# modassarrana89/authorino

Hardware: AMD Instinct MI355X
Metric: request×rule evals/sec (+ allow/deny decisions/sec, % HBM roofline) (higher is better)
Workload: dtype u8

## Files before the change

authorino_amd/csrc/ajx_api.cpp:

```cpp
#include <cstdio>
#include <cstring>
#include <memory>
#include <string>

#include "ajx_host.h"
#include "ajx_blob.h"
#include "ajx_kernels.h"

thread_local AjxLastError ajx_last_error;

struct EndEvent {
    hipEvent_t ev = nullptr;
    ~EndEvent() {
        if (ev) (void)hipEventDestroy(ev);
    }
};

struct Workspace {
    hipStream_t stream = nullptr;
    uint64_t id = 0;
    uint32_t refs = 0;
    bool retired = false;
    std::mutex mu;
    hipEvent_t ev0 = nullptr, ev1 = nullptr;
    std::shared_ptr<EndEvent> end;
    const uint8_t** d_sets = nullptr;
    ajx::DeviceBuf sets_dev;
    ajx::PinnedBuf sets_host;
    uint32_t sets_cap = 0;
    uint32_t sets_slot = 0;
    hipEvent_t sets_ev[2] = {nullptr, nullptr};
    bool sets_ev_rec[2] = {false, false};
    std::vector<const uint8_t*> last_sets;
    ajx::PtrTable progs;
    ajx::DeviceBuf slow;
    bool cnt_zero = false, exact_published = false;
    ajx::DeviceBuf rows;
    ajx::DeviceBuf perm;
    ajx::DeviceBuf tout;
    const authjx_ruleset* rows_rs = nullptr;
    uint32_t rows_n = 0, rows_stride = 0;
    const uint32_t* rows_perm = nullptr;
    bool rows_wave = false;
    bool ran = false;
};

namespace {
std::mutex g_reg_mu;
std::vector<std::pair<uint64_t, std::shared_ptr<EndEvent>>> g_reg;
uint64_t g_next_ws = 1;

Workspace* workspace_of(authjx_ctx* ctx, hipStream_t s) {
    for (Workspace* w : ctx->ws)
        if (w->stream == s) return w;
    Workspace* w = new Workspace();
    w->stream = s;
    w->end = std::make_shared<EndEvent>();
    if (hipEventCreate(&w->ev0) != hipSuccess || hipEventCreate(&w->end->ev) != hipSuccess) {
        if (w->ev0) (void)hipEventDestroy(w->ev0);
        delete w;
        return nullptr;
    }
    w->ev1 = w->end->ev;
    {
        std::lock_guard<std::mutex> lock(g_reg_mu);
        w->id = g_next_ws++;
        g_reg.push_back({w->id, w->end});
    }
    ctx->ws.push_back(w);
    return w;
}

void destroy_workspace(Workspace* w) {
    if (w->ran) (void)hipEventSynchronize(w->ev1);
    {
        std::lock_guard<std::mutex> lock(g_reg_mu);
        for (size_t i = 0; i < g_reg.size(); i++)
            if (g_reg[i].first == w->id) {
                g_reg.erase(g_reg.begin() + (long)i);
                break;
            }
    }
    for (int k = 0; k < 2; k++) {
        if (w->sets_ev[k]) (void)hipEventDestroy(w->sets_ev[k]);
        if (w->progs.ev[k]) (void)hipEventDestroy(w->progs.ev[k]);
    }
    if (w->ev0) (void)hipEventDestroy(w->ev0);
    delete w;
}

Workspace* ws_ref(Workspace* w) {
// ... 3 lines not shown
void ws_unref(authjx_ctx* ctx, Workspace* w) {
    bool dead;
    {
        std::lock_guard<std::mutex> g(ctx->mu);
        dead = --w->refs == 0 && w->retired;
    }
    if (dead) destroy_workspace(w);
}

int ensure_sets(Workspace* w, int device, const authjx_ruleset* const* sets, uint32_t n_sets,
                const uint8_t* const* d_pre = nullptr) {
    std::vector<const uint8_t*> ptrs(n_sets);
    for (uint32_t i = 0; i < n_sets; i++) {
        if (!sets[i] || sets[i]->device != device) return AUTHJX_EINVAL;
        ptrs[i] = sets[i]->d_blob.data();
    }
    if (d_pre) {
        w->d_sets = const_cast<const uint8_t**>(d_pre);
        w->last_sets.clear();
        return AUTHJX_OK;
    }
    if (ptrs == w->last_sets) return AUTHJX_OK;
    if (n_sets > w->sets_cap) {
        const uint32_t cap = n_sets < 64 ? 64 : n_sets;
        w->d_sets = nullptr;
        w->sets_cap = 0;
        w->sets_ev_rec[0] = w->sets_ev_rec[1] = false;
        HIP_OK(w->sets_dev.reserve(2 * cap * sizeof(uint8_t*), w->stream));
        HIP_OK(w->sets_host.reserve(2 * cap * sizeof(uint8_t*), w->stream));
        for (int k = 0; k < 2; k++)
            if (!w->sets_ev[k]) HIP_OK(hipEventCreateWithFlags(&w->sets_ev[k], hipEventDisableTiming));
        w->sets_cap = cap;
    }
    const uint32_t k = w->d_sets ? 1u - w->sets_slot : 0u;
    if (w->sets_ev_rec[k]) HIP_OK(hipEventSynchronize(w->sets_ev[k]));
    const uint8_t** h = w->sets_host.as<const uint8_t*>() + (size_t)k * w->sets_cap;
    const uint8_t** dv = w->sets_dev.as<const uint8_t*>() + (size_t)k * w->sets_cap;
    std::memcpy(h, ptrs.data(), n_sets * sizeof(uint8_t*));
    HIP_OK(hipMemcpyAsync(dv, h, n_sets * sizeof(uint8_t*), hipMemcpyHostToDevice, w->stream));
    w->sets_slot = k;
    w->d_sets = dv;
    w->last_sets = ptrs;
    return AUTHJX_OK;
}

int ensure_work(Workspace* w, uint32_t n, uint32_t row_stride) {
    const size_t slow_bytes = ((size_t)n + ajx::kStreamCounterWords) * sizeof(uint32_t);
    const size_t perm_bytes = ajx::PermBuf::words(n) * sizeof(uint32_t);
    const size_t rows_bytes = (size_t)((n + 63u) & ~63u) * row_stride * sizeof(uint64_t);
    if (slow_bytes <= w->slow.capacity() && perm_bytes <= w->perm.capacity() && rows_bytes <= w->rows.capacity())
        return AUTHJX_OK;
    w->rows_rs = nullptr;
    if (slow_bytes > w->slow.capacity()) w->cnt_zero = w->exact_published = false;
    HIP_OK(w->slow.reserve(slow_bytes, w->stream));
    HIP_OK(w->perm.reserve(perm_bytes, w->stream));
    HIP_OK(w->rows.reserve(rows_bytes, w->stream));
    return AUTHJX_OK;
}

struct WsLock {
    authjx_ctx* ctx;
    Workspace* w = nullptr;
    std::unique_lock<std::mutex> lock;
    WsLock(authjx_ctx* c, void* stream) : ctx(c) {
        {
            std::lock_guard<std::mutex> g(ctx->mu);
            w = ws_ref(workspace_of(ctx, stream ? (hipStream_t)stream : ctx->stream));
        }
        if (w) {
            lock = std::unique_lock<std::mutex>(w->mu);
            std::lock_guard<std::mutex> g(ctx->mu);
            if (!w->retired) ctx->last_ws = w;
        }
    }
    ~WsLock() {
        if (!w) return;
        lock.unlock();
        ws_unref(ctx, w);
    }
    WsLock(const WsLock&) = delete;
    WsLock& operator=(const WsLock&) = delete;
};

struct LastWs {
    authjx_ctx* ctx;
    Workspace* w = nullptr;
    int force_scan = 0;
    explicit LastWs(authjx_ctx* c) : ctx(c) {
        std::lock_guard<std::mutex> g(ctx->mu);
        w = ws_ref(ctx->last_ws);
        force_scan = ctx->force_scan;
    }
    ~LastWs() {
        if (w) ws_unref(ctx, w);
    }
    LastWs(const LastWs&) = delete;
    LastWs& operator=(const LastWs&) = delete;
};

int batch_done(Workspace* w, const authjx_ruleset* const* sets, uint32_t n_sets) {
    HIP_OK(hipEventRecord(w->ev1, w->stream));
    if (w->sets_ev[w->sets_slot]) {
        HIP_OK(hipEventRecord(w->sets_ev[w->sets_slot], w->stream));
        w->sets_ev_rec[w->sets_slot] = true;
    }
    w->ran = true;
    for (uint32_t i = 0; i < n_sets; i++) const_cast<authjx_ruleset*>(sets[i])->note_use(w->id);
    return AUTHJX_OK;
}
// ... 120 lines not shown
    ajx::PtrTable& t = w->progs;
    if (t.last.empty() || !std::equal(t.last.begin(), t.last.end(), ptrs, ptrs + n)) {
        if (n > t.cap) {
            const uint32_t cap = n < 64 ? 64 : n;
            t.cap = 0;
            t.last.clear();
            t.rec[0] = t.rec[1] = false;
            HIP_OK(t.dev.reserve(2 * (size_t)cap * sizeof(uint8_t*), w->stream));
            HIP_OK(t.host.reserve(2 * (size_t)cap * sizeof(uint8_t*), w->stream));
            for (int k = 0; k < 2; k++)
                if (!t.ev[k]) HIP_OK(hipEventCreateWithFlags(&t.ev[k], hipEventDisableTiming));
            t.cap = cap;
        }
        const uint32_t k = t.last.empty() ? 0u : 1u - t.slot;
        if (t.rec[k]) HIP_OK(hipEventSynchronize(t.ev[k]));
        const uint8_t** h = t.host.as<const uint8_t*>() + (size_t)k * t.cap;
        std::memcpy(h, ptrs, n * sizeof(uint8_t*));
        HIP_OK(hipMemcpyAsync(t.dev.as<const uint8_t*>() + (size_t)k * t.cap, h, n * sizeof(uint8_t*),
                              hipMemcpyHostToDevice, w->stream));
        t.slot = k;
        t.last.assign(ptrs, ptrs + n);
    }
    HIP_OK(launch(t.dev.as<const uint8_t*>() + (size_t)t.slot * t.cap, w->stream));
    HIP_OK(hipEventRecord(t.ev[t.slot], w->stream));
    t.rec[t.slot] = true;
    HIP_OK(hipEventRecord(w->ev1, w->stream));
    w->ran = true;
    return AUTHJX_OK;
}

int eval_device(authjx_ctx* ctx, const authjx_ruleset* const* sets, uint32_t n_sets, const uint32_t* d_set_of_req,
                const uint8_t* d_arena, const uint64_t* d_offs, const uint32_t* d_lens, uint32_t n,
                uint8_t* d_out_tristate, int32_t* d_out_err_idx, uint64_t* d_out_bitmap, uint32_t bitmap_stride_words,
                void* stream, const uint8_t* const* d_sets_pre) {
    if (!ctx || !sets || n_sets == 0 || (n && (!d_arena || !d_offs || !d_lens || !d_out_tristate)))
        return AUTHJX_EINVAL;
    if (n_sets > 1 && !d_set_of_req) return AUTHJX_EINVAL;
    if (n_sets == 1) d_set_of_req = nullptr;
    uint32_t need_words = 0;
    for (uint32_t i = 0; i < n_sets; i++) {
        if (!sets[i] || sets[i]->c.n_trees != sets[0]->c.n_trees) return AUTHJX_EINVAL;
        need_words = std::max(need_words, (sets[i]->c.n_patterns + 63) / 64);
    }
    if (d_out_bitmap && bitmap_stride_words < need_words) return AUTHJX_EINVAL;
    const ajx::PlanIn in = plan_in(ctx, sets, n_sets, n, d_out_bitmap != nullptr);
    const ajx::EvalPlan plan = ajx::plan_eval(in);
    WsLock wl(ctx, stream);
    Workspace* w = wl.w;
    if (!w) return AUTHJX_EDEVICE;
    hipStream_t s = w->stream;
    HIP_OK(hipSetDevice(ctx->device));
    int rc = ensure_sets(w, ctx->device, sets, n_sets, d_sets_pre);
    if (rc != AUTHJX_OK) return rc;
    if (plan.path != ajx::kPathExact && (rc = ensure_work(w, n, plan.rows_stride)) != AUTHJX_OK) return rc;
    HIP_OK(hipEventRecord(w->ev0, s));
    w->rows_rs = plan.keep_rows ? sets[0] : nullptr;
    w->rows_n = n;
    w->rows_stride = plan.rows_stride;
    w->rows_perm = nullptr;
    w->rows_wave = true;
    bool cnt_zero = w->cnt_zero;
    w->cnt_zero = w->exact_published = false;
    uint32_t* const slow = w->slow.as<uint32_t>();
    const ajx::Batch batch{w->d_sets, d_set_of_req, d_arena, d_offs, d_lens, n};
    const ajx::Results res{d_out_tristate, d_out_err_idx, d_out_bitmap, bitmap_stride_words};
    if (plan.path == ajx::kPathExact) {
        HIP_OK(ajx::launch_eval_scan(batch, res, plan.mods != 0, s));
    } else if (plan.path == ajx::kPathStream) {
        const ajx::Work work{w->rows.as<uint64_t>(), plan.rows_stride, slow, ajx::stream_slow_ids(slow)};
        HIP_OK(ajx::launch_eval_stream(batch, res, work, plan, in.max_blob, in.max_rec,
                                       ajx::PermBuf{w->perm.as<uint32_t>(), n}.stage_list(), &cnt_zero, s));
        w->cnt_zero = w->exact_published = cnt_zero;
    } else {
        const uint32_t* perm = nullptr;
        uint32_t* pos_of = nullptr;
        const ajx::PermBuf order{w->perm.as<uint32_t>(), n};
        if (plan.len_order) {
            if (plan.want_pos_of) {
                HIP_OK(w->tout.reserve(ajx::tout_bytes(n, plan.n_out, plan.tout_bm ? bitmap_stride_words : 0u), s));
                pos_of = order.pos_of();
            }
            HIP_OK(ajx::launch_len_order(d_lens, n, order.hist(), order.perm(), pos_of, s));
            perm = order.perm();
        }
        w->rows_perm = perm;
        const ajx::Work work{w->rows.as<uint64_t>(), plan.rows_stride, slow, slow + 1};
        HIP_OK(ajx::launch_eval_fast(batch, res, work, plan, perm, pos_of, pos_of ? w->tout.data() : nullptr, s));
    }
    return batch_done(w, sets, n_sets);
}

extern "C" {

#ifndef AJX_SRC_HASH
#define AJX_SRC_HASH "unknown"
#endif
const char* authjx_build_hash(void) { return AJX_SRC_HASH; }

int authjx_device_count(void) {
    int n = 0;
    if (hipGetDeviceCount(&n) != hipSuccess) return 0;
    return n;
}

int authjx_init(int device, authjx_ctx** out) {
    if (!out) return AUTHJX_EINVAL;
    *out = nullptr;
    int n = authjx_device_count();
    if (device < 0 || device >= n) return AUTHJX_EDEVICE;
    HIP_OK(hipSetDevice(device));
    authjx_ctx* c = new authjx_ctx();
    c->device = device;
    if (hipStreamCreateWithFlags(&c->stream, hipStreamNonBlocking) != hipSuccess) {
        delete c;
        return AUTHJX_EDEVICE;
    }
    *out = c;
    return AUTHJX_OK;
}

void authjx_shutdown(authjx_ctx* ctx) {
    if (!ctx) return;
    std::vector<authjx_batcher*> live;
    {
        std::lock_guard<std::mutex> g(ctx->mu);
        live = ctx->batchers;
    }
    for (authjx_batcher* b : live) authjx_batcher_destroy(b);
    (void)hipSetDevice(ctx->device);
    if (ctx->stream) (void)hipStreamSynchronize(ctx->stream);
    for (Workspace* w : ctx->ws) destroy_workspace(w);
    if (ctx->stream) (void)hipStreamDestroy(ctx->stream);
    delete ctx;
}

int authjx_release_stream(authjx_ctx* ctx, void* stream) {
    if (!ctx || !stream || (hipStream_t)stream == ctx->stream) return AUTHJX_EINVAL;
    (void)hipSetDevice(ctx->device);
    retire_stream(ctx, (hipStream_t)stream);
    return AUTHJX_OK;
}

// ... 37 lines not shown
}

uint32_t authjx_ruleset_patterns(const authjx_ruleset* rs) { return rs ? rs->c.n_patterns : 0; }
uint32_t authjx_ruleset_selectors(const authjx_ruleset* rs) { return rs ? rs->c.n_selectors : 0; }

size_t authjx_pattern_error(const authjx_ruleset* rs, uint32_t i, char* buf, size_t cap) {
    if (!rs || i >= rs->c.n_patterns) return 0;
    const std::string& e = rs->c.pattern_error[i];
    if (buf && cap) std::snprintf(buf, cap, "%s", e.c_str());
    return e.size();
}

int authjx_eval_batch_device(authjx_ctx* ctx, const authjx_ruleset* const* sets, uint32_t n_sets,
                             const uint32_t* d_set_of_req, const uint8_t* d_arena, const uint64_t* d_offs,
                             const uint32_t* d_lens, uint32_t n, uint8_t* d_out_tristate, int32_t* d_out_err_idx,
                             uint64_t* d_out_bitmap, uint32_t bitmap_stride_words, void* stream) {
    return eval_device(ctx, sets, n_sets, d_set_of_req, d_arena, d_offs, d_lens, n, d_out_tristate, d_out_err_idx,
                       d_out_bitmap, bitmap_stride_words, stream, nullptr);
}

static_assert(sizeof(authjx_value) == 12, "authjx_value is three u32 words on the device");

int authjx_select_batch_device(authjx_ctx* ctx, const authjx_ruleset* const* sets, uint32_t n_sets,
                               const uint32_t* d_set_of_req, const uint8_t* d_arena, const uint64_t* d_offs,
                               const uint32_t* d_lens, uint32_t n, authjx_value* d_out_values,
                               uint32_t values_stride, void* stream) {
    return authjx_select_text_batch_device(ctx, sets, n_sets, d_set_of_req, d_arena, d_offs, d_lens, n, d_out_values,
                                           values_stride, nullptr, 0, stream);
}

int authjx_select_text_batch_device(authjx_ctx* ctx, const authjx_ruleset* const* sets, uint32_t n_sets,
                                    const uint32_t* d_set_of_req, const uint8_t* d_arena, const uint64_t* d_offs,
                                    const uint32_t* d_lens, uint32_t n, authjx_value* d_out_values,
                                    uint32_t values_stride, uint8_t* d_out_text, uint32_t text_stride, void* stream) {
    if (!ctx || !sets || n_sets == 0 || (n && (!d_arena || !d_offs || !d_lens || !d_out_values)))
        return AUTHJX_EINVAL;
    if (d_out_text && text_stride == 0) return AUTHJX_EINVAL;
    if (n_sets > 1 && !d_set_of_req) return AUTHJX_EINVAL;
    if (n_sets == 1) d_set_of_req = nullptr;
    for (uint32_t i = 0; i < n_sets; i++)
        if (!sets[i] || sets[i]->c.n_patterns > values_stride) return AUTHJX_EINVAL;
    const ajx::PlanIn in = plan_in(ctx, sets, n_sets, n, false);
    const uint32_t row_stride = 1 + in.max_sel;
    WsLock wl(ctx, stream);
    Workspace* w = wl.w;
    if (!w) return AUTHJX_EDEVICE;
    hipStream_t s = w->stream;
    HIP_OK(hipSetDevice(ctx->device));
    int rc = ensure_sets(w, ctx->device, sets, n_sets);
    if (rc != AUTHJX_OK) return rc;
    const bool exact = in.force_scan != 0;
    w->rows_rs = nullptr;
    w->cnt_zero = w->exact_published = false;
    if (!exact && (rc = ensure_work(w, n, row_stride)) != AUTHJX_OK) return rc;
    const uint32_t* perm = nullptr;
    if (!exact && in.len_sort && n_sets == 1 && n >= 4096) {
        const ajx::PermBuf order{w->perm.as<uint32_t>(), n};
        HIP_OK(ajx::launch_len_order(d_lens, n, order.hist(), order.perm(), nullptr, s));
        perm = order.perm();
    }
    const uint32_t shared_bytes =
        (n_sets == 1 && sets[0]->blob_bytes <= ajx::kMaxSharedBlobBytes) ? sets[0]->blob_bytes : 0u;
    uint32_t* const slow = w->slow.as<uint32_t>();
    const ajx::Batch batch{w->d_sets, d_set_of_req, d_arena, d_offs, d_lens, n};
    const ajx::Values values{reinterpret_cast<uint32_t*>(d_out_values), values_stride, d_out_text, text_stride};
    const ajx::Work work{exact ? nullptr : w->rows.as<uint64_t>(), row_stride, slow, slow + 1};
    HIP_OK(ajx::launch_select(batch, shared_bytes, values, work, perm, s));
    return batch_done(w, sets, n_sets);
}

int authjx_select_from_eval_device(authjx_ctx* ctx, const authjx_ruleset* rs, uint32_t first_pattern,
                                   const uint8_t* d_arena, const uint64_t* d_offs, const uint32_t* d_lens,
                                   uint32_t n, authjx_value* d_out_values, uint32_t values_stride, void* stream) {
    if (!ctx || !rs || values_stride == 0 || (n && (!d_arena || !d_offs || !d_lens || !d_out_values)))
        return AUTHJX_EINVAL;
    if (first_pattern + values_stride > rs->c.n_patterns) return AUTHJX_EINVAL;
    WsLock wl(ctx, stream);
    Workspace* w = wl.w;
    if (!w) return AUTHJX_EDEVICE;
    if (w->rows_rs != rs || w->rows_n != n || !rows_hold_patterns(rs, first_pattern, values_stride))
        return AUTHJX_EINVAL;
    hipStream_t s = w->stream;
    HIP_OK(hipSetDevice(ctx->device));
    const authjx_ruleset* one[1] = {rs};
    int rc = ensure_sets(w, ctx->device, one, 1);
    if (rc != AUTHJX_OK) return rc;
    const ajx::Batch batch{w->d_sets, nullptr, d_arena, d_offs, d_lens, n};
    const ajx::Values values{reinterpret_cast<uint32_t*>(d_out_values), values_stride, nullptr, 0};
    const ajx::Work work{w->rows.as<uint64_t>(), w->rows_stride, nullptr, nullptr};
    HIP_OK(ajx::launch_select_rows(batch, values, work, first_pattern, w->rows_perm, w->rows_wave, s));
    return batch_done(w, one, 1);
}

int authjx_select_batch(authjx_ctx* ctx, const authjx_ruleset* const* sets, uint32_t n_sets,
                        const uint32_t* set_of_req, const uint8_t* arena, uint64_t arena_len,
                        const uint64_t* offs, const uint32_t* lens, uint32_t n, authjx_value* out_values,
                        uint32_t values_stride) {
    return authjx_select_text_batch(ctx, sets, n_sets, set_of_req, arena, arena_len, offs, lens, n, out_values,
                                    values_stride, nullptr, 0);
}

int authjx_select_text_batch(authjx_ctx* ctx, const authjx_ruleset* const* sets, uint32_t n_sets,
                             const uint32_t* set_of_req, const uint8_t* arena, uint64_t arena_len,
                             const uint64_t* offs, const uint32_t* lens, uint32_t n, authjx_value* out_values,
                             uint32_t values_stride, uint8_t* out_text, uint32_t text_stride) {
    if (!ctx || (n && (!arena || !offs || !lens || !out_values))) return AUTHJX_EINVAL;
    if (out_text && text_stride == 0) return AUTHJX_EINVAL;
    if (!host_batch_ok(offs, lens, set_of_req, n, arena_len, n_sets)) return AUTHJX_EINVAL;
    const size_t out_bytes = (size_t)n * values_stride * sizeof(authjx_value);
    const size_t text_bytes = out_text ? (size_t)n * text_stride : 0;
    ajx::StageLayout lay;
    const StagedIn in = lay_inputs(lay, arena_len, n, set_of_req != nullptr);
    const size_t o_out = lay.add(out_bytes), o_text = lay.add(text_bytes);
    std::lock_guard<std::mutex> batch_lock(ctx->batch_mu);
    int rc = upload_inputs(ctx, lay.total(), in, arena, arena_len, offs, lens, set_of_req, n);
    if (rc != AUTHJX_OK) return rc;
    uint8_t* b = ctx->stage.data();
    rc = authjx_select_text_batch_device(ctx, sets, n_sets, set_of_req ? (const uint32_t*)(b + in.sor) : nullptr, b,
                                         (const uint64_t*)(b + in.offs), (const uint32_t*)(b + in.lens), n,
                                         (authjx_value*)(b + o_out), values_stride, out_text ? b + o_text : nullptr,
                                         text_stride, nullptr);
// ... 119 lines not shown
```

authorino_amd/csrc/ajx_kernels.hip:

```cpp
#include <hip/hip_runtime.h>

#include <atomic>

#include "ajx_fast.h"
#include "ajx_modifiers.h"
#include "ajx_stream_body.h"
#include "ajx_kernels.h"
#include "ajx_kcommon.h"

namespace ajx {

template <bool MODS>
__global__ __launch_bounds__(256) void ajx_eval_scan(const uint8_t* const* __restrict__ sets,
                                                     const uint32_t* __restrict__ set_of_req,
                                                     const uint8_t* __restrict__ arena,
                                                     const uint64_t* __restrict__ offs,
                                                     const uint32_t* __restrict__ lens, uint32_t n,
                                                     uint8_t* __restrict__ out_tri, int32_t* __restrict__ out_err,
                                                     uint64_t* __restrict__ out_bm, uint32_t stride) {
    const uint32_t r = blockIdx.x * blockDim.x + threadIdx.x;
    if (r >= n) return;
    if constexpr (MODS) {
        ModBufs mb;
        eval_scan_one<true>(r, sets, set_of_req, arena, offs, lens, out_tri, out_err, out_bm, stride, &mb);
    } else {
        eval_scan_one<false>(r, sets, set_of_req, arena, offs, lens, out_tri, out_err, out_bm, stride, nullptr);
    }
}

template <bool MODS>
__global__ __launch_bounds__(256) void ajx_eval_scan_list(const uint8_t* const* __restrict__ sets,
                                                          const uint32_t* __restrict__ set_of_req,
                                                          const uint8_t* __restrict__ arena,
                                                          const uint64_t* __restrict__ offs,
                                                          const uint32_t* __restrict__ lens,
                                                          const uint32_t* __restrict__ slow_count,
                                                          const uint32_t* __restrict__ slow_ids,
                                                          uint8_t* __restrict__ out_tri, int32_t* __restrict__ out_err,
                                                          uint64_t* __restrict__ out_bm, uint32_t stride) {
    const uint32_t cnt = *slow_count;
    if constexpr (MODS) {
        ModBufs mb;
        for (uint32_t i = blockIdx.x * blockDim.x + threadIdx.x; i < cnt; i += gridDim.x * blockDim.x)
            eval_scan_one<true>(slow_ids[i], sets, set_of_req, arena, offs, lens, out_tri, out_err, out_bm, stride,
                                &mb);
    } else {
        for (uint32_t i = blockIdx.x * blockDim.x + threadIdx.x; i < cnt; i += gridDim.x * blockDim.x)
            eval_scan_one<false>(slow_ids[i], sets, set_of_req, arena, offs, lens, out_tri, out_err, out_bm, stride,
                                 nullptr);
    }
}

static void launch_slow_list(const Batch& b, const Results& res, const Work& work, bool mods, uint32_t sgrid,
                             hipStream_t stream) {
    hipLaunchKernelGGL((mods ? ajx_eval_scan_list<true> : ajx_eval_scan_list<false>), dim3(sgrid), dim3(256), 0, stream,
                       b.sets, b.set_of_req, b.arena, b.offs, b.lens, work.slow_count, work.slow_ids, res.tri, res.err,
                       res.bm, res.stride);
}
// ... 209 lines not shown
        return hipSuccess;
    });
    if (e != hipSuccess) return e;
#define AJX_STREAM_LAUNCH(M, T, LT, F)                                                                           \
    hipLaunchKernelGGL((ajx_scan_stream<M, T, LT, F>), dim3(grid), dim3(block), lds, stream, b.sets, b.set_of_req, \
                       b.arena, b.offs, b.lens, n, ctr, work.slow_ids, d_stage_ids, res.tri, res.err, res.bm,      \
                       res.stride, wave_off, wave_bytes, work.rows, work.row_stride,                                \
                       (keep_rows ? kKeepRows : 0u) | (timing ? kKeepTiming : 0u), per, merge ? 1u : 0u)
    const bool lat = merge && !keep_rows;
    const bool fin = lat && !mods && n <= kFinMaxN;
    if (mt && fin)
        AJX_STREAM_LAUNCH(0, true, true, true);
    else if (mt && lat)
        AJX_STREAM_LAUNCH(0, true, true, false);
    else if (mt)
        AJX_STREAM_LAUNCH(0, true, false, false);
    else if (mode == 1)
        AJX_STREAM_LAUNCH(1, false, false, false);
    else if (mode == 2)
        AJX_STREAM_LAUNCH(2, false, false, false);
    else if (fin)
        AJX_STREAM_LAUNCH(0, false, true, true);
    else if (lat)
        AJX_STREAM_LAUNCH(0, false, true, false);
    else
        AJX_STREAM_LAUNCH(0, false, false, false);
#undef AJX_STREAM_LAUNCH
    if ((e = hipGetLastError()) != hipSuccess) return e;
    if (counters_zero) *counters_zero = fin && (mt || (mode != 1 && mode != 2));
    if (mode != 0 || fin) return hipSuccess;
    const uint32_t fgrid = n < 2048u * 256u ? (n + 255) / 256 : 4096;
#define AJX_FINISH_LAUNCH(T, X, LDS)                                                                            \
    hipLaunchKernelGGL((ajx_stream_finish<T, X>), dim3(fgrid), dim3(256), LDS, stream, b.sets,                     \
                       T ? b.set_of_req : nullptr, b.arena, b.offs, b.lens, d_stage_ids, work.rows,                \
                       work.row_stride, ctr, work.slow_ids, res.tri, res.err, res.bm, res.stride)
    if (mt && mods)
        AJX_FINISH_LAUNCH(true, 2, 0);
    else if (mt)
        AJX_FINISH_LAUNCH(true, 1, 0);
    else if (merge && mods)
        AJX_FINISH_LAUNCH(false, 2, wave_off);
    else if (merge)
        AJX_FINISH_LAUNCH(false, 1, wave_off);
    else
        AJX_FINISH_LAUNCH(false, 0, wave_off);
#undef AJX_FINISH_LAUNCH
    if ((e = hipGetLastError()) != hipSuccess) return e;
    if (merge) return hipSuccess;
    const uint32_t sgrid = n < 1024u * 128u ? 2 * ((n + 255) / 256) : 4096;
    launch_slow_list(b, res, work, mods, sgrid, stream);
    return hipGetLastError();
}

constexpr uint32_t kLenBuckets = 1024;

__device__ __forceinline__ uint32_t len_bucket(uint32_t len) {
    const uint32_t b = len >> 3;
    return kLenBuckets - 1u - (b < kLenBuckets ? b : kLenBuckets - 1u);
}

__global__ __launch_bounds__(kLenBuckets) void ajx_len_hist(const uint32_t* __restrict__ lens, uint32_t n,
                                                            uint32_t* __restrict__ hist) {
    __shared__ uint32_t h[kLenBuckets];
    h[threadIdx.x] = 0;
    __syncthreads();
    for (uint32_t i = blockIdx.x * blockDim.x + threadIdx.x; i < n; i += gridDim.x * blockDim.x)
        atomicAdd(&h[len_bucket(lens[i])], 1u);
    __syncthreads();
    if (h[threadIdx.x]) atomicAdd(&hist[threadIdx.x], h[threadIdx.x]);
}

constexpr uint32_t kLenSpreadMin = 32;
__global__ __launch_bounds__(kLenBuckets) void ajx_len_scan(const uint32_t* __restrict__ hist,
                                                            uint32_t* __restrict__ cursor) {
    __shared__ uint32_t s[kLenBuckets];
    __shared__ uint32_t lo, hi;
    const uint32_t t = threadIdx.x;
    const uint32_t own = hist[t];
    if (t == 0) {
        lo = kLenBuckets;
        hi = 0;
    }
    s[t] = own;
    __syncthreads();
    if (own) {
        atomicMin(&lo, t);
        atomicMax(&hi, t);
    }
    for (uint32_t o = 1; o < kLenBuckets; o <<= 1) {
        const uint32_t v = t >= o ? s[t - o] : 0u;
        __syncthreads();
        s[t] += v;
        __syncthreads();
    }
    cursor[t] = s[t] - own;
    if (t == 0) cursor[kLenBuckets] = (hi < lo || hi - lo < kLenSpreadMin) ? 1u : 0u;
}

__global__ __launch_bounds__(kLenBuckets) void ajx_len_scatter(const uint32_t* __restrict__ lens, uint32_t n,
                                                               uint32_t* __restrict__ cursor,
                                                               uint32_t* __restrict__ perm,
                                                               uint32_t* __restrict__ pos_of) {
    __shared__ uint32_t cnt[kLenBuckets];
    __shared__ uint32_t base[kLenBuckets];
    const uint32_t i = blockIdx.x * blockDim.x + threadIdx.x;
    if (cursor[kLenBuckets]) {
        if (i < n) {
            perm[i] = i;
            if (pos_of) pos_of[i] = i;
        }
        return;
    }
    cnt[threadIdx.x] = 0;
    __syncthreads();
    uint32_t b = 0, rank = 0;
    if (i < n) {
        b = len_bucket(lens[i]);
        rank = atomicAdd(&cnt[b], 1u);
    }
    __syncthreads();
    if (cnt[threadIdx.x]) base[threadIdx.x] = atomicAdd(&cursor[threadIdx.x], cnt[threadIdx.x]);
    __syncthreads();
    if (i < n) {
        perm[base[b] + rank] = i;
        if (pos_of) pos_of[i] = base[b] + rank;
    }
}

__global__ __launch_bounds__(256) void ajx_unpermute(const uint32_t* __restrict__ pos_of, uint32_t n, uint32_t n_out,
                                                     uint32_t stride, const uint8_t* __restrict__ t_tri,
                                                     const int32_t* __restrict__ t_err,
                                                     const uint64_t* __restrict__ t_bm, uint8_t* __restrict__ tri,
                                                     int32_t* __restrict__ err, uint64_t* __restrict__ bm) {
    const uint32_t i = blockIdx.x * blockDim.x + threadIdx.x;
    if (i >= n) return;
    const size_t j = pos_of[i];
    for (uint32_t q = 0; q < n_out; q++) {
        tri[(size_t)i * n_out + q] = t_tri[j * n_out + q];
        if (err) err[(size_t)i * n_out + q] = t_err[j * n_out + q];
    }
    if (bm)
        for (uint32_t w = 0; w < stride; w++) bm[(size_t)i * stride + w] = t_bm[j * stride + w];
}

hipError_t launch_len_order(const uint32_t* d_lens, uint32_t n, uint32_t* d_hist, uint32_t* d_perm,
                            uint32_t* d_pos_of, hipStream_t stream) {
    hipError_t e = hipMemsetAsync(d_hist, 0, (2 * kLenBuckets + 1) * sizeof(uint32_t), stream);
    if (e != hipSuccess) return e;
    const uint32_t blocks = (n + kLenBuckets - 1) / kLenBuckets;
    hipLaunchKernelGGL(ajx_len_hist, dim3(blocks < 512 ? blocks : 512), dim3(kLenBuckets), 0, stream, d_lens, n,
                       d_hist);
    hipLaunchKernelGGL(ajx_len_scan, dim3(1), dim3(kLenBuckets), 0, stream, d_hist, d_hist + kLenBuckets);
    hipLaunchKernelGGL(ajx_len_scatter, dim3(blocks), dim3(kLenBuckets), 0, stream, d_lens, n, d_hist + kLenBuckets,
                       d_perm, d_pos_of);
    return hipGetLastError();
}

template <bool TEXT>
__global__ __launch_bounds__(256) void ajx_select_values(const uint8_t* const* __restrict__ sets,
                                                         const uint32_t* __restrict__ set_of_req,
                                                         const uint8_t* __restrict__ arena,
                                                         const uint64_t* __restrict__ offs,
                                                         const uint32_t* __restrict__ lens, uint32_t n,
                                                         uint32_t* __restrict__ out, uint32_t stride,
                                                         const uint64_t* __restrict__ rows, uint32_t row_stride,
                                                         uint32_t p0, const uint32_t* __restrict__ perm,
                                                         uint32_t wave_rows, uint8_t* __restrict__ text,
                                                         uint32_t text_stride) {
    const uint32_t k = blockIdx.x * blockDim.x + threadIdx.x;
    if (k >= n) return;
    const uint32_t r = perm ? perm[k] : k;
    select_request<TEXT>(r, k, sets, set_of_req, arena, offs, lens, out, stride, rows, row_stride, p0, wave_rows, text,
                         text_stride);
}

hipError_t launch_select(const Batch& b, uint32_t shared_blob_bytes, const Values& v, const Work& work,
                         const uint32_t* d_perm, hipStream_t stream) {
    const uint32_t n = b.n;
    if (n == 0) return hipSuccess;
    if (work.rows) {
        const bool shared = shared_blob_bytes != 0 && b.set_of_req == nullptr;
        const uint32_t fblock = shared ? fast_block(shared_blob_bytes) : kFastBlock;
        const uint32_t fgrid = (n + fblock - 1) / fblock;
        const RingGeom g = ring_geom(shared ? shared_blob_bytes : 0u, fblock);
        hipError_t e = hipMemsetAsync(work.slow_count, 0, sizeof(uint32_t), stream);
        if (e != hipSuccess) return e;
        static std::atomic<uint64_t> attr_done{0};
        e = attr_once(attr_done, [] {
            const void* ks[] = {reinterpret_cast<const void*>(&ajx_scan_fast<true>),
                                reinterpret_cast<const void*>(&ajx_scan_fast<false>)};
            for (const void* k : ks) {
                const hipError_t r = hipFuncSetAttribute(k, hipFuncAttributeMaxDynamicSharedMemorySize, 160 * 1024);
                if (r != hipSuccess) return r;
            }
            return hipSuccess;
        });
        if (e != hipSuccess) return e;
        hipLaunchKernelGGL((shared ? ajx_scan_fast<true> : ajx_scan_fast<false>), dim3(fgrid), dim3(fblock), g.lds,
                           stream, b.sets, b.set_of_req, b.arena, b.offs, b.lens, n, work.rows, work.row_stride,
                           work.slow_count, work.slow_ids, g.ring_off, d_perm);
        if ((e = hipGetLastError()) != hipSuccess) return e;
    }
    const uint32_t block = 256;
    const uint32_t grid = (n + block - 1) / block;
    hipLaunchKernelGGL((v.text ? ajx_select_values<true> : ajx_select_values<false>), dim3(grid), dim3(block), 0, stream,
                       b.sets, b.set_of_req, b.arena, b.offs, b.lens, n, v.out, v.stride, work.rows, work.row_stride, 0u,
                       nullptr, 0u, v.text, v.text ? v.text_stride : 0u);
// ... 69 lines not shown
```

authorino_amd/csrc/ajx_plan.h:

```cpp
#pragma once
#include <stdint.h>

namespace ajx {

constexpr uint32_t kMaxSharedBlobBytes = 48 * 1024;
constexpr uint32_t kMaxTenantStageBytes = 16 * 1024;
constexpr uint32_t kStreamSpan = 32;

struct StreamCounters {
    uint32_t slow;
    uint32_t stage_b;
    uint32_t waves_done;
    uint32_t exact_published;
};
constexpr uint32_t kStreamCounterWords = sizeof(StreamCounters) / sizeof(uint32_t);
inline StreamCounters* stream_counters(uint32_t* slow_buf) { return reinterpret_cast<StreamCounters*>(slow_buf); }
inline uint32_t* stream_slow_ids(uint32_t* slow_buf) { return slow_buf + kStreamCounterWords; }

constexpr uint32_t kPermHistWords = 4096;
struct PermBuf {
    uint32_t* p;
    uint32_t n;
    static constexpr uint64_t words(uint32_t n) { return 2ull * n + kPermHistWords; }
    uint32_t* perm() const { return p; }
    uint32_t* hist() const { return p + n; }
    uint32_t* pos_of() const { return p + n + kPermHistWords; }
    uint32_t* stage_list() const { return p; }
};

enum KernelMode : int {
    kModeDefault = 0,
    kModeLeanLoads = 15, kModeLeanClassify, kModeLeanWalk, kModeLeanStageA,
    kModeBare = 40,
    kModeLeanForStream = 41,
    kModeStreamStructural = 50,
    kModeStreamNoFold = 51,
    kModeStreamAnyN = 52,
    kModeStreamClocks = 53,
};

inline bool mode_lean_ablation(int m) { return m >= kModeLeanLoads && m <= kModeLeanStageA; }
inline bool mode_known(int m) {
    return m == kModeDefault || mode_lean_ablation(m) || m == kModeBare || m == kModeLeanForStream ||
           (m >= kModeStreamStructural && m <= kModeStreamClocks);
}

struct PlanIn {
    uint32_t n, n_sets;
    uint32_t all_stream;
    uint32_t max_rec, max_sel, max_blob;
    uint32_t n_trees, lean_feat;
    uint32_t mods;
    uint32_t bitmap;
    int32_t force_scan, mode, len_sort, no_tenant_stage;
    uint32_t stream_max_n;
};

enum Path : uint32_t {
    kPathExact,
    kPathStream,
    kPathLean,
    kPathTenant,
    kPathFused,
    kPathInvalid,
};
enum StreamMode : uint32_t { kStreamFull, kStreamStructural, kStreamNoFold, kStreamTiming };

struct EvalPlan {
    uint32_t path;
    uint32_t stream_mode;
    uint32_t per;
    uint32_t abl;
    uint32_t keep_rows;
    uint32_t rows_stride;
    uint32_t stage_bytes;
    uint32_t len_order;
    uint32_t want_pos_of;
    uint32_t out_k;
    uint32_t tout_bm;
    uint32_t n_out;
// ... 52 lines not shown
```

Measured before the change: 15.64 billion.

## Fuse length-order histogram and scan via last-block ticket, self-zeroing region

```diff
diff --git a/authorino_amd/csrc/ajx_api.cpp b/authorino_amd/csrc/ajx_api.cpp
--- a/authorino_amd/csrc/ajx_api.cpp
+++ b/authorino_amd/csrc/ajx_api.cpp
@@ -37,6 +37,7 @@
     bool cnt_zero = false, exact_published = false;
     ajx::DeviceBuf rows;
     ajx::DeviceBuf perm;
+    bool order_dirty = true;
     ajx::DeviceBuf tout;
     const authjx_ruleset* rows_rs = nullptr;
     uint32_t rows_n = 0, rows_stride = 0;
@@ -146,9 +147,37 @@
         return AUTHJX_OK;
     w->rows_rs = nullptr;
     if (slow_bytes > w->slow.capacity()) w->cnt_zero = w->exact_published = false;
+    if (perm_bytes > w->perm.capacity()) w->order_dirty = true;
     HIP_OK(w->slow.reserve(slow_bytes, w->stream));
     HIP_OK(w->perm.reserve(perm_bytes, w->stream));
     HIP_OK(w->rows.reserve(rows_bytes, w->stream));
+    return AUTHJX_OK;
+}
+
+struct OrderGuard {
+    Workspace* w;
+    bool ok = false;
+    explicit OrderGuard(Workspace* ws) : w(ws) {}
+    ~OrderGuard() {
+        if (!ok) w->order_dirty = true;
+    }
+    int done(int rc) {
+        ok = rc == AUTHJX_OK;
+        return rc;
+    }
+};
+
+int len_order(Workspace* w, const uint32_t* d_lens, uint32_t n, bool want_pos_of, const uint32_t** perm,
+              uint32_t** pos_of) {
+    const ajx::PermBuf order{w->perm.as<uint32_t>(), n};
+    if (w->order_dirty) {
+        HIP_OK(hipMemsetAsync(order.hist(), 0, ajx::kPermHistWords * sizeof(uint32_t), w->stream));
+        w->order_dirty = false;
+    }
+    uint32_t* const inv = want_pos_of ? order.pos_of() : nullptr;
+    HIP_OK(ajx::launch_len_order(d_lens, n, order.hist(), order.perm(), inv, w->stream));
+    *perm = order.perm();
+    if (pos_of) *pos_of = inv;
     return AUTHJX_OK;
 }
 
@@ -375,6 +404,7 @@
     HIP_OK(hipSetDevice(ctx->device));
     int rc = ensure_sets(w, ctx->device, sets, n_sets, d_sets_pre);
     if (rc != AUTHJX_OK) return rc;
+    OrderGuard og(w);
     if (plan.path != ajx::kPathExact && (rc = ensure_work(w, n, plan.rows_stride)) != AUTHJX_OK) return rc;
     HIP_OK(hipEventRecord(w->ev0, s));
     w->rows_rs = plan.keep_rows ? sets[0] : nullptr;
@@ -397,20 +427,16 @@
     } else {
         const uint32_t* perm = nullptr;
         uint32_t* pos_of = nullptr;
-        const ajx::PermBuf order{w->perm.as<uint32_t>(), n};
         if (plan.len_order) {
-            if (plan.want_pos_of) {
+            if (plan.want_pos_of)
                 HIP_OK(w->tout.reserve(ajx::tout_bytes(n, plan.n_out, plan.tout_bm ? bitmap_stride_words : 0u), s));
-                pos_of = order.pos_of();
-            }
-            HIP_OK(ajx::launch_len_order(d_lens, n, order.hist(), order.perm(), pos_of, s));
-            perm = order.perm();
+            if ((rc = len_order(w, d_lens, n, plan.want_pos_of != 0, &perm, &pos_of)) != AUTHJX_OK) return rc;
         }
         w->rows_perm = perm;
         const ajx::Work work{w->rows.as<uint64_t>(), plan.rows_stride, slow, slow + 1};
         HIP_OK(ajx::launch_eval_fast(batch, res, work, plan, perm, pos_of, pos_of ? w->tout.data() : nullptr, s));
     }
-    return batch_done(w, sets, n_sets);
+    return og.done(batch_done(w, sets, n_sets));
 }
 
 extern "C" {
@@ -554,13 +580,12 @@
     const bool exact = in.force_scan != 0;
     w->rows_rs = nullptr;
     w->cnt_zero = w->exact_published = false;
+    OrderGuard og(w);
     if (!exact && (rc = ensure_work(w, n, row_stride)) != AUTHJX_OK) return rc;
     const uint32_t* perm = nullptr;
-    if (!exact && in.len_sort && n_sets == 1 && n >= 4096) {
-        const ajx::PermBuf order{w->perm.as<uint32_t>(), n};
-        HIP_OK(ajx::launch_len_order(d_lens, n, order.hist(), order.perm(), nullptr, s));
-        perm = order.perm();
-    }
+    if (!exact && in.len_sort && n_sets == 1 && n >= 4096 &&
+        (rc = len_order(w, d_lens, n, false, &perm, nullptr)) != AUTHJX_OK)
+        return rc;
     const uint32_t shared_bytes =
         (n_sets == 1 && sets[0]->blob_bytes <= ajx::kMaxSharedBlobBytes) ? sets[0]->blob_bytes : 0u;
     uint32_t* const slow = w->slow.as<uint32_t>();
@@ -568,7 +593,7 @@
     const ajx::Values values{reinterpret_cast<uint32_t*>(d_out_values), values_stride, d_out_text, text_stride};
     const ajx::Work work{exact ? nullptr : w->rows.as<uint64_t>(), row_stride, slow, slow + 1};
     HIP_OK(ajx::launch_select(batch, shared_bytes, values, work, perm, s));
-    return batch_done(w, sets, n_sets);
+    return og.done(batch_done(w, sets, n_sets));
 }
 
 int authjx_select_from_eval_device(authjx_ctx* ctx, const authjx_ruleset* rs, uint32_t first_pattern,
diff --git a/authorino_amd/csrc/ajx_kernels.hip b/authorino_amd/csrc/ajx_kernels.hip
--- a/authorino_amd/csrc/ajx_kernels.hip
+++ b/authorino_amd/csrc/ajx_kernels.hip
@@ -4,6 +4,7 @@
 
 #include "ajx_fast.h"
 #include "ajx_modifiers.h"
+#include "ajx_order.h"
 #include "ajx_stream_body.h"
 #include "ajx_kernels.h"
 #include "ajx_kcommon.h"
@@ -319,79 +320,55 @@
     return hipGetLastError();
 }
 
-constexpr uint32_t kLenBuckets = 1024;
-
-__device__ __forceinline__ uint32_t len_bucket(uint32_t len) {
-    const uint32_t b = len >> 3;
-    return kLenBuckets - 1u - (b < kLenBuckets ? b : kLenBuckets - 1u);
-}
-
-__global__ __launch_bounds__(kLenBuckets) void ajx_len_hist(const uint32_t* __restrict__ lens, uint32_t n,
-                                                            uint32_t* __restrict__ hist) {
-    __shared__ uint32_t h[kLenBuckets];
-    h[threadIdx.x] = 0;
-    __syncthreads();
-    for (uint32_t i = blockIdx.x * blockDim.x + threadIdx.x; i < n; i += gridDim.x * blockDim.x)
-        atomicAdd(&h[len_bucket(lens[i])], 1u);
-    __syncthreads();
-    if (h[threadIdx.x]) atomicAdd(&hist[threadIdx.x], h[threadIdx.x]);
-}
-
-constexpr uint32_t kLenSpreadMin = 32;
-__global__ __launch_bounds__(kLenBuckets) void ajx_len_scan(const uint32_t* __restrict__ hist,
-                                                            uint32_t* __restrict__ cursor) {
-    __shared__ uint32_t s[kLenBuckets];
-    __shared__ uint32_t lo, hi;
+
+__global__ __launch_bounds__(order::kBlock) void ajx_len_hist(const uint32_t* __restrict__ lens, uint32_t n,
+                                                              uint32_t* __restrict__ region) {
+    __shared__ order::Lds s;
     const uint32_t t = threadIdx.x;
-    const uint32_t own = hist[t];
-    if (t == 0) {
-        lo = kLenBuckets;
-        hi = 0;
-    }
-    s[t] = own;
-    __syncthreads();
-    if (own) {
-        atomicMin(&lo, t);
-        atomicMax(&hi, t);
-    }
-    for (uint32_t o = 1; o < kLenBuckets; o <<= 1) {
-        const uint32_t v = t >= o ? s[t - o] : 0u;
+    order::clear(s, t);
+    __syncthreads();
+    order::hist_count(s, lens, n, blockIdx.x, gridDim.x, t);
+    __syncthreads();
+    order::hist_publish(s, region, t);
+    __syncthreads();
+    order::ticket(s, region, order::kTicketHist, gridDim.x, t);
+    __syncthreads();
+    if (!s.last) return;
+    const uint32_t own = order::scan_load(s, region, t);
+    __syncthreads();
+    order::scan_range(s, own, t);
+    for (uint32_t o = 1; o < order::kLenBuckets; o <<= 1) {
+        const uint32_t v = order::scan_read(s, o, t);
         __syncthreads();
-        s[t] += v;
+        order::scan_add(s, v, t);
         __syncthreads();
     }
-    cursor[t] = s[t] - own;
-    if (t == 0) cursor[kLenBuckets] = (hi < lo || hi - lo < kLenSpreadMin) ? 1u : 0u;
-}
-
-__global__ __launch_bounds__(kLenBuckets) void ajx_len_scatter(const uint32_t* __restrict__ lens, uint32_t n,
-                                                               uint32_t* __restrict__ cursor,
-                                                               uint32_t* __restrict__ perm,
-                                                               uint32_t* __restrict__ pos_of) {
-    __shared__ uint32_t cnt[kLenBuckets];
-    __shared__ uint32_t base[kLenBuckets];
-    const uint32_t i = blockIdx.x * blockDim.x + threadIdx.x;
-    if (cursor[kLenBuckets]) {
-        if (i < n) {
-            perm[i] = i;
-            if (pos_of) pos_of[i] = i;
-        }
-        return;
-    }
-    cnt[threadIdx.x] = 0;
-    __syncthreads();
-    uint32_t b = 0, rank = 0;
-    if (i < n) {
-        b = len_bucket(lens[i]);
-        rank = atomicAdd(&cnt[b], 1u);
-    }
-    __syncthreads();
-    if (cnt[threadIdx.x]) base[threadIdx.x] = atomicAdd(&cursor[threadIdx.x], cnt[threadIdx.x]);
-    __syncthreads();
-    if (i < n) {
-        perm[base[b] + rank] = i;
-        if (pos_of) pos_of[i] = base[b] + rank;
-    }
+    order::scan_store(s, region, own, t);
+}
+
+template <uint32_t ITEMS>
+__global__ __launch_bounds__(order::kBlock) void ajx_len_scatter(const uint32_t* __restrict__ lens, uint32_t n,
+                                                                 uint32_t* __restrict__ region,
+                                                                 uint32_t* __restrict__ perm,
+                                                                 uint32_t* __restrict__ pos_of) {
+    __shared__ order::Lds s;
+    const uint32_t t = threadIdx.x;
+    if (order::scatter_narrow(region)) {
+        order::scatter_identity<ITEMS>(n, perm, pos_of, blockIdx.x, t);
+    } else {
+        order::clear(s, t);
+        __syncthreads();
+        order::ScatterThread<ITEMS> st;
+        order::scatter_rank(s, lens, n, st, blockIdx.x, t);
+        __syncthreads();
+        order::scatter_base(s, region, t);
+        __syncthreads();
+        order::scatter_store(s, n, st, perm, pos_of, blockIdx.x, t);
+    }
+    __syncthreads();
+    order::ticket(s, region, order::kTicketScatter, gridDim.x, t);
+    __syncthreads();
+    if (s.last) order::region_zero(region, t);
 }
 
 __global__ __launch_bounds__(256) void ajx_unpermute(const uint32_t* __restrict__ pos_of, uint32_t n, uint32_t n_out,
@@ -410,16 +387,16 @@
         for (uint32_t w = 0; w < stride; w++) bm[(size_t)i * stride + w] = t_bm[j * stride + w];
 }
 
+static_assert(order::kRegionWords <= kPermHistWords, "the order's region fits the order buffer's");
+
 hipError_t launch_len_order(const uint32_t* d_lens, uint32_t n, uint32_t* d_hist, uint32_t* d_perm,
                             uint32_t* d_pos_of, hipStream_t stream) {
-    hipError_t e = hipMemsetAsync(d_hist, 0, (2 * kLenBuckets + 1) * sizeof(uint32_t), stream);
-    if (e != hipSuccess) return e;
-    const uint32_t blocks = (n + kLenBuckets - 1) / kLenBuckets;
-    hipLaunchKernelGGL(ajx_len_hist, dim3(blocks < 512 ? blocks : 512), dim3(kLenBuckets), 0, stream, d_lens, n,
-                       d_hist);
-    hipLaunchKernelGGL(ajx_len_scan, dim3(1), dim3(kLenBuckets), 0, stream, d_hist, d_hist + kLenBuckets);
-    hipLaunchKernelGGL(ajx_len_scatter, dim3(blocks), dim3(kLenBuckets), 0, stream, d_lens, n, d_hist + kLenBuckets,
-                       d_perm, d_pos_of);
+    if (n == 0) return hipSuccess;
+    hipLaunchKernelGGL(ajx_len_hist, dim3(order::hist_grid(n)), dim3(order::kBlock), 0, stream, d_lens, n, d_hist);
+    const uint32_t items = order::scatter_items(n);
+    hipLaunchKernelGGL((items == 1 ? ajx_len_scatter<1> : ajx_len_scatter<order::kScatterItemsLarge>),
+                       dim3(order::scatter_grid(n, items)), dim3(order::kBlock), 0, stream, d_lens, n, d_hist, d_perm,
+                       d_pos_of);
     return hipGetLastError();
 }
 
diff --git a/authorino_amd/csrc/ajx_order.h b/authorino_amd/csrc/ajx_order.h
--- /dev/null
+++ b/authorino_amd/csrc/ajx_order.h
@@ -0,0 +1,165 @@
+#pragma once
+#include <stdint.h>
+
+#if defined(__HIPCC__)
+#define AJX_ORD __device__ __forceinline__
+#else
+#define AJX_ORD inline
+#endif
+
+namespace ajx {
+namespace order {
+
+constexpr uint32_t kLenBuckets = 1024;
+constexpr uint32_t kLenSpreadMin = 32;
+constexpr uint32_t kBlock = kLenBuckets;
+constexpr uint32_t kFlag = kLenBuckets, kTicketHist = kLenBuckets + 1, kTicketScatter = kLenBuckets + 2;
+constexpr uint32_t kRegionWords = kLenBuckets + 3;
+
+#if defined(__HIPCC__)
+AJX_ORD uint32_t add(uint32_t* p, uint32_t v) { return atomicAdd(p, v); }
+AJX_ORD void umin(uint32_t* p, uint32_t v) { atomicMin(p, v); }
+AJX_ORD void umax(uint32_t* p, uint32_t v) { atomicMax(p, v); }
+AJX_ORD void fence_release() { __builtin_amdgcn_fence(__ATOMIC_RELEASE, "agent"); }
+AJX_ORD void fence_acquire() { __builtin_amdgcn_fence(__ATOMIC_ACQUIRE, "agent"); }
+AJX_ORD void drain() { asm volatile("s_waitcnt vmcnt(0)" ::: "memory"); }
+AJX_ORD uint32_t load_fresh(const uint32_t* p) { return __hip_atomic_load(p, __ATOMIC_RELAXED, __HIP_MEMORY_SCOPE_AGENT); }
+#else
+inline uint32_t add(uint32_t* p, uint32_t v) {
+    const uint32_t o = *p;
+    *p = o + v;
+    return o;
+}
+inline void umin(uint32_t* p, uint32_t v) {
+    if (v < *p) *p = v;
+}
+inline void umax(uint32_t* p, uint32_t v) {
+    if (v > *p) *p = v;
+}
+inline void fence_release() {}
+inline void fence_acquire() {}
+inline void drain() {}
+inline uint32_t load_fresh(const uint32_t* p) { return *p; }
+#endif
+
+#if defined(__HIPCC__)
+__host__
+#endif
+AJX_ORD uint32_t len_bucket(uint32_t len) {
+    const uint32_t b = len >> 3;
+    return kLenBuckets - 1u - (b < kLenBuckets ? b : kLenBuckets - 1u);
+}
+
+constexpr uint32_t kHistMaxGrid = 128;
+inline uint32_t hist_grid(uint32_t n) {
+    const uint32_t blocks = (n + kBlock - 1) / kBlock;
+    return blocks < kHistMaxGrid ? blocks : kHistMaxGrid;
+}
+constexpr uint32_t kScatterItemsLarge = 8;
+constexpr uint32_t kScatterLargeMin = 64u * 1024u;
+inline uint32_t scatter_items(uint32_t n) { return n > kScatterLargeMin ? kScatterItemsLarge : 1u; }
+inline uint32_t scatter_grid(uint32_t n, uint32_t items) { return (n + kBlock * items - 1) / (kBlock * items); }
+
+struct Lds {
+    uint32_t cnt[kLenBuckets];
+    uint32_t base[kLenBuckets];
+    uint32_t lo, hi, last;
+};
+
+AJX_ORD void clear(Lds& s, uint32_t t) { s.cnt[t] = 0; }
+
+AJX_ORD void ticket(Lds& s, uint32_t* region, uint32_t word, uint32_t grid, uint32_t t) {
+    if (t == 0) {
+        fence_release();
+        drain();
+        s.last = add(&region[word], 1u) + 1u == grid ? 1u : 0u;
+        if (s.last) fence_acquire();
+    }
+}
+
+AJX_ORD void hist_count(Lds& s, const uint32_t* lens, uint32_t n, uint32_t block, uint32_t grid, uint32_t t) {
+    for (uint32_t i = block * kBlock + t; i < n; i += grid * kBlock) add(&s.cnt[len_bucket(lens[i])], 1u);
+}
+AJX_ORD void hist_publish(const Lds& s, uint32_t* region, uint32_t t) {
+    if (s.cnt[t]) add(&region[t], s.cnt[t]);
+    drain();
+}
+AJX_ORD uint32_t scan_load(Lds& s, const uint32_t* region, uint32_t t) {
+    const uint32_t own = load_fresh(&region[t]);
+    s.cnt[t] = own;
+    if (t == 0) {
+        s.lo = kLenBuckets;
+        s.hi = 0;
+    }
+    return own;
+}
+AJX_ORD void scan_range(Lds& s, uint32_t own, uint32_t t) {
+    if (own) {
+        umin(&s.lo, t);
+        umax(&s.hi, t);
+    }
+}
+AJX_ORD uint32_t scan_read(const Lds& s, uint32_t o, uint32_t t) { return t >= o ? s.cnt[t - o] : 0u; }
+AJX_ORD void scan_add(Lds& s, uint32_t v, uint32_t t) { s.cnt[t] += v; }
+AJX_ORD void scan_store(const Lds& s, uint32_t* region, uint32_t own, uint32_t t) {
+    region[t] = s.cnt[t] - own;
+    if (t == 0) region[kFlag] = (s.hi < s.lo || s.hi - s.lo < kLenSpreadMin) ? 1u : 0u;
+}
+
+template <uint32_t ITEMS>
+struct ScatterThread {
+    uint32_t b[ITEMS], rank[ITEMS];
+};
+
+AJX_ORD bool scatter_narrow(const uint32_t* region) { return region[kFlag] != 0; }
+
+template <uint32_t ITEMS>
+AJX_ORD void scatter_identity(uint32_t n, uint32_t* perm, uint32_t* pos_of, uint32_t block, uint32_t t) {
+#pragma unroll
+    for (uint32_t k = 0; k < ITEMS; k++) {
+        const uint32_t i = (block * ITEMS + k) * kBlock + t;
+        if (i < n) {
+            perm[i] = i;
+            if (pos_of) pos_of[i] = i;
+        }
+    }
+}
+template <uint32_t ITEMS>
+AJX_ORD void scatter_rank(Lds& s, const uint32_t* lens, uint32_t n, ScatterThread<ITEMS>& st, uint32_t block,
+                          uint32_t t) {
+#pragma unroll
+    for (uint32_t k = 0; k < ITEMS; k++) {
+        const uint32_t i = (block * ITEMS + k) * kBlock + t;
+        st.b[k] = i < n ? len_bucket(lens[i]) : 0u;
+    }
+#pragma unroll
+    for (uint32_t k = 0; k < ITEMS; k++) {
+        const uint32_t i = (block * ITEMS + k) * kBlock + t;
+        st.rank[k] = i < n ? add(&s.cnt[st.b[k]], 1u) : 0u;
+    }
+}
+AJX_ORD void scatter_base(Lds& s, uint32_t* region, uint32_t t) {
+    if (s.cnt[t]) s.base[t] = add(&region[t], s.cnt[t]);
+    drain();
+}
+template <uint32_t ITEMS>
+AJX_ORD void scatter_store(const Lds& s, uint32_t n, const ScatterThread<ITEMS>& st, uint32_t* perm,
+                           uint32_t* pos_of, uint32_t block, uint32_t t) {
+#pragma unroll
+    for (uint32_t k = 0; k < ITEMS; k++) {
+        const uint32_t i = (block * ITEMS + k) * kBlock + t;
+        if (i >= n) continue;
+        const uint32_t pos = s.base[st.b[k]] + st.rank[k];
+        if (pos < n) {
+            perm[pos] = i;
+            if (pos_of) pos_of[i] = pos;
+        }
+    }
+}
+AJX_ORD void region_zero(uint32_t* region, uint32_t t) {
+    region[t] = 0;
+    if (t == 0) region[kFlag] = region[kTicketHist] = region[kTicketScatter] = 0;
+}
+
+}
+}
diff --git a/authorino_amd/csrc/ajx_plan.h b/authorino_amd/csrc/ajx_plan.h
--- a/authorino_amd/csrc/ajx_plan.h
+++ b/authorino_amd/csrc/ajx_plan.h
@@ -22,10 +22,10 @@
     uint32_t* p;
     uint32_t n;
     static constexpr uint64_t words(uint32_t n) { return 2ull * n + kPermHistWords; }
-    uint32_t* perm() const { return p; }
-    uint32_t* hist() const { return p + n; }
-    uint32_t* pos_of() const { return p + n + kPermHistWords; }
-    uint32_t* stage_list() const { return p; }
+    uint32_t* hist() const { return p; }
+    uint32_t* perm() const { return p + kPermHistWords; }
+    uint32_t* pos_of() const { return p + kPermHistWords + n; }
+    uint32_t* stage_list() const { return p + kPermHistWords; }
 };
 
 enum KernelMode : int {
```

Measured after the change: 15.79 billion, median of 6. Within noise of the previous version (+1.0%).
